# seshnadathur/victor

Measured on AMD Instinct MI355X. Metric: likelihood evals/sec (40 s-bins, 100 mu, l=0,2,4), higher is better.
Workload: dtype f64

## Files before the change

### victor_amd/csrc/vk_devmath.h

```cpp
#pragma once

#include <hip/hip_runtime.h>

namespace vkm {

template <int CTRL, int ROW_MASK, bool BOUND_CTRL = false>
__device__ __forceinline__ double dpp_move(double v) {
  int lo = __double2loint(v), hi = __double2hiint(v);
  lo = __builtin_amdgcn_update_dpp(0, lo, CTRL, ROW_MASK, 0xF, BOUND_CTRL);
  hi = __builtin_amdgcn_update_dpp(0, hi, CTRL, ROW_MASK, 0xF, BOUND_CTRL);
  return __hiloint2double(hi, lo);
}

__device__ __forceinline__ double wave_sum(double v) {
  v += dpp_move<0xB1, 0xF, true>(v);
  v += dpp_move<0x4E, 0xF, true>(v);
  v += dpp_move<0x141, 0xF, true>(v);
  v += dpp_move<0x140, 0xF, true>(v);
  v += dpp_move<0x142, 0xF, true>(v);
  v += dpp_move<0x143, 0xF, true>(v);
  const int lo = __builtin_amdgcn_readlane(__double2loint(v), 63);
  const int hi = __builtin_amdgcn_readlane(__double2hiint(v), 63);
  return __hiloint2double(hi, lo);
}

__device__ __forceinline__ double fold32(double x, double y) {
  const auto lo = __builtin_amdgcn_permlane32_swap((unsigned)__double2loint(x), (unsigned)__double2loint(y), false, false);
  const auto hi = __builtin_amdgcn_permlane32_swap((unsigned)__double2hiint(x), (unsigned)__double2hiint(y), false, false);
  return __hiloint2double((int)hi[0], (int)lo[0]) + __hiloint2double((int)hi[1], (int)lo[1]);
}
__device__ __forceinline__ double fold16(double x, double y) {
  const auto lo = __builtin_amdgcn_permlane16_swap((unsigned)__double2loint(x), (unsigned)__double2loint(y), false, false);
  const auto hi = __builtin_amdgcn_permlane16_swap((unsigned)__double2hiint(x), (unsigned)__double2hiint(y), false, false);
  return __hiloint2double((int)hi[0], (int)lo[0]) + __hiloint2double((int)hi[1], (int)lo[1]);
}
__device__ __forceinline__ double octet_sum(double v) {
  v += dpp_move<0x141, 0xF, true>(v);
  v += dpp_move<0xB1, 0xF, true>(v);
  v += dpp_move<0x4E, 0xF, true>(v);
  return v;
}

__device__ __forceinline__ void sqrt_rsqrt(double x, double& g, double& ir) {
  const double y = __builtin_amdgcn_rsq(x);
  const double e = fma(-(x * y), y, 1.0);
  const double p = fma(0.375, e, 0.5);
  ir = fma(y * e, p, y);
  g = x * ir;
}

__device__ __forceinline__ double rsqrt3(double x) {
  const double y = __builtin_amdgcn_rsq(x);
  const double e = fma(-(x * y), y, 1.0);
  const double p = fma(0.375, e, 0.5);
  return fma(y * e, p, y);
}

__device__ __forceinline__ double rsqrt_nr(double x) {
  const double y = __builtin_amdgcn_rsq(x);
  const double e = fma(-(x * y), y, 1.0);
  return fma(y * e, 0.5, y);
}

__device__ __forceinline__ double recip(double x) {
  const double y = __builtin_amdgcn_rcp(x);
  const double e = fma(-x, y, 1.0);
  return fma(y, fma(e, e, e), y);
}

constexpr int kExpNonposTab = 256;
__device__ __forceinline__ double exp2_frac(int j) { return exp2((double)j * (1.0 / kExpNonposTab)); }

__device__ __forceinline__ double fma3(double p, double f, double c) {
  double r;
  asm("v_fma_f64 %0, %1, %2, %3" : "=v"(r) : "v"(p), "v"(f), "v"(c));
  return r;
}

__device__ __forceinline__ double exp_nonpos(double a, const double* __restrict__ tab) {
  a = fmax(a, -750.0);
  const double n = rint(a * 369.3299304675746);
  double f = fma(n, -0x1.62e42fee00000p-9, a);
  f = fma(n, -0x1.a39ef35793c76p-41, f);
  const int ni = (int)n;
  const double t = tab[ni & (kExpNonposTab - 1)];
  double p = fma3(f, 1.0 / 24.0, 1.0 / 6.0);
  p = fma(p, f, 0.5);
  p = fma(p, f, 1.0);
  p = fma(p, f, 1.0);
  return ldexp(t * p, ni >> 8);
}

__device__ __forceinline__ double fma_s(double p, double f, double c) {
  double r;
  asm("v_fma_f64 %0, %1, %2, %3" : "=v"(r) : "v"(p), "v"(f), "s"(c));
  return r;
}

__device__ __forceinline__ double recip_nr(double x) {
  const double y = __builtin_amdgcn_rcp(x);
  const double e = fma(-x, y, 1.0);
  return fma(y, e, y);
}

__device__ __forceinline__ void recip_shared2(double a, double b, double& ra, double& rb) {
  const double P = a * b;
  const double y = recip(P);
  ra = y * b;
  rb = y * a;
}
__device__ __forceinline__ void recip_shared3(double a, double b, double c, double& ra, double& rb, double& rc) {
  const double ab = a * b;
  const double P = ab * c;
  const double y = recip(P);
  const double yc = y * c;
  rc = y * ab;
  ra = yc * b;
  rb = yc * a;
}
__device__ __forceinline__ void recip_shared4(double a, double b, double c, double d, double& ra, double& rb, double& rc, double& rd) {
  const double ab = a * b, cd = c * d;
  const double P = ab * cd;
  const double y = recip(P);
  const double yab = y * ab;
  const double ycd = y * cd;
  ra = ycd * b;
  rb = ycd * a;
  rc = yab * d;
  rd = yab * c;
}

__device__ __forceinline__ double rsqrt_nr_x2(double x) {
  const double y = __builtin_amdgcn_rsq(x);
  const double h = x * y;
  const double w = fma(-h, y, 3.0);
  return y * w;
}

__device__ __forceinline__ double rsqrt3_x2(double x) {
  const double y = __builtin_amdgcn_rsq(x);
  const double e = fma(-(x * y), y, 1.0);
  const double p2 = fma(0.75, e, 1.0);
  return y * fma(e, p2, 2.0);
}

constexpr double kExpScale = 13.589148804608305 * 0x1p-9;
constexpr double kExpC = 709.782712893383996843;
template <int EXPT> struct ExpCfg;
template <> struct ExpCfg<0> {
  static constexpr int kBits = 8, kEntries = 256, kDoubles = 256, kDegree = 3;
  static constexpr double kMagic = 0x1.8p34;
  static constexpr double kLead = kExpC * kExpC * kExpC / 6.0;
};
template <> struct ExpCfg<1> {
  static constexpr int kBits = 6, kEntries = 64, kDoubles = 64 * 32, kDegree = 4;
  static constexpr double kMagic = 0x1.8p36;
  static constexpr double kLead = kExpC * kExpC * kExpC * kExpC / 24.0;
};
constexpr int kExpTab = ExpCfg<0>::kDoubles;

template <int EXPT>
__device__ __forceinline__ double exp_table_entry(int j) {
  typedef ExpCfg<EXPT> C;
  const double t = C::kLead * exp2((double)j * (1.0 / C::kEntries));
  return __hiloint2double(__double2hiint(t) - (j << (20 - C::kBits)), __double2loint(t));
}
template <int EXPT>
__device__ __forceinline__ double exp_table_slot(int e) { return exp_table_entry<EXPT>(EXPT == 1 ? (e >> 5) : e); }

__device__ __forceinline__ void clamp_keeps_nan() { asm volatile("s_setreg_imm32_b32 hwreg(HW_REG_MODE, 8, 1), 0"); }

template <int EXPT>
__device__ __forceinline__ double exp_gauss(double ynum, double inv_sv, const double* __restrict__ tab, unsigned lane_off = 0) {
  typedef ExpCfg<EXPT> C;
  double yp;
  asm("v_mul_f64 %0, |%1|, |%2| clamp" : "=v"(yp) : "v"(ynum), "v"(inv_sv));
  const double nd = fma(-yp, yp, C::kMagic);
  const double nn = nd - C::kMagic;
  const double d = fma(-yp, yp, -nn);
  const int n = __double2loint(nd);
  unsigned off;
  if (EXPT == 0) {
    asm("v_lshlrev_b32_sdwa %0, %1, %2 dst_sel:DWORD dst_unused:UNUSED_PAD src0_sel:DWORD src1_sel:BYTE_0" : "=v"(off) : "v"(3), "v"(n));
    __builtin_assume(off < 2048u);
  } else {
    asm("v_and_b32 %0, 63, %1\n\tv_lshl_or_b32 %0, %0, 8, %2" : "=&v"(off) : "v"(n), "v"(lane_off));
  }
  (void)tab;
  double t;
  asm("ds_read_b64 %0, %1\n\ts_waitcnt lgkmcnt(0)" : "=v"(t) : "v"(off));
  const double ts = __hiloint2double(__double2hiint(t) + (n << (20 - C::kBits)), __double2loint(t));
  double q;
  if (C::kDegree == 3) {
    q = d + 3.0 / kExpC;
    q = fma_s(q, d, 6.0 / (kExpC * kExpC));
    q = fma_s(q, d, 6.0 / (kExpC * kExpC * kExpC));
  } else {
    q = d + 4.0 / kExpC;
    q = fma_s(q, d, 12.0 / (kExpC * kExpC));
    q = fma_s(q, d, 24.0 / (kExpC * kExpC * kExpC));
    q = fma_s(q, d, 24.0 / (kExpC * kExpC * kExpC * kExpC));
  }
  return ts * q;
}

}
```

### victor_amd/csrc/vk_kernel_cells.h

```cpp
#pragma once
#include "vk_kernel_fast.h"

namespace vk {

struct CellsPlan {
  int mu, w, s, betar, da, v1, sva, image_end, acc, like, total;
};

__host__ __device__ inline int cells_range_bins(int n_mu, int cpi) { return (cpi + n_mu - 2) / n_mu + 1; }

__host__ __device__ inline CellsPlan make_cells_plan(int n_mu, int n_x, int n_s, int uni_n, int nlr, int n_beta_r,
                                                     int lut_n, int with_da, int cpi, int n_like, int n_sva = 0) {
  CellsPlan p;
  int o = fast_fixed_doubles(uni_n, nlr, lut_n);
  o = (o + 1) & ~1;
  p.mu = o;    o += 2 * n_mu;
  p.w = o;     o += kMaxEll * n_mu;
  p.s = o;     o += (n_s + 1) & ~1;
  p.betar = o; o += (n_beta_r + 1) & ~1;
  p.da = o;    o += with_da ? uni_n * 4 : 0;
  p.v1 = o;    o += with_da == 1 ? 0 : uni_n * 4;
  o = (o + 1) & ~1;
  p.sva = o;   o += (n_sva + 1) & ~1;
  p.image_end = o;
  int bins = cells_range_bins(n_mu, cpi);
  if (bins > n_s) bins = n_s;
  p.acc = o;   o += kMaxEll * (bins + 1) * kWaves;
  o = (o + 1) & ~1;
  p.like = o;  o += n_like > 0 ? like_lds_doubles(n_like) : 0;
  p.total = o;
  return p;
}

template <int NLR>
__device__ __forceinline__ void stage_cells(const TheoryArgs& a, const CellsPlan& pl, double* lds, int with_da) {
  const int tid = threadIdx.x;
  for (int i = tid; i < a.n_mu; i += kBlock) {
    const double m = a.mu[i];
    lds[pl.mu + 2 * i] = m;
    lds[pl.mu + 2 * i + 1] = sqrt(1.0 - m * m);
#pragma unroll
    for (int l = 0; l < kMaxEll; ++l) lds[pl.w + l * a.n_mu + i] = (l < a.n_ell) ? a.w_ell[l * a.n_mu + i] : 0.0;
  }
  for (int j = tid; j < a.n_s; j += kBlock) lds[pl.s + j] = a.s[j];
  stage_uni_records<NLR>(a, lds);
  if (with_da) stage_da<NLR>(a, lds + pl.da);
  if (with_da != 1) for (int e = tid; e < a.uni_n * 4; e += kBlock) lds[pl.v1 + e] = a.uni_sv_v[(e >> 2) * 8 + 4 + (e & 3)];
  if (a.n_beta_r > 0)
    for (int i = tid; i < a.n_beta_r; i += kBlock) lds[pl.betar + i] = a.beta_r[i];
  if (pl.image_end > pl.sva)
    for (int e = tid; e < a.sva_doubles; e += kBlock) lds[pl.sva + e] = a.sva[e];
}

template <int NL>
__device__ __forceinline__ void finish_point_ranges(const TheoryArgs& a, long long point, double beta, double poison, double* th,
                                                    bool gather, const double* lds_beta_r) {
  const int N = a.n_ell * a.n_s;
  const double w0 = a.wsum[0], w1 = a.wsum[1], w2 = a.wsum[2];
  const bool keep_out = !a.fuse || a.want_theory;
  LikePrefetch<kLikeRowsCells> pf;
  if (a.fuse) pf.issue(a.like, beta, late_tid(), lds_beta_r);
  for (int e = late_tid(); gather && e < N; e += kBlock) {
    const int l = (e >= 2 * a.n_s) ? 2 : (e >= a.n_s ? 1 : 0), j = e - l * a.n_s;
    const int q_first = (j * a.n_mu) / a.cells_per_item, q_last = (j * a.n_mu + a.n_mu - 1) / a.cells_per_item;
    double part[8];
    load_shared_x8(partial_slot(a, point, l, j), part);
    double v = 0.0;
#pragma unroll
    for (int c = 0; c < kMaxParts; ++c) v += (c <= q_last - q_first) ? part[c] : 0.0;
    v = v - (l == 0 ? w0 : (l == 1 ? w1 : w2)) + poison;
    if (keep_out) a.out[point * (long long)N + e] = v;
    th[e] = v;
  }
  __syncthreads();
  if (a.fuse) like_point_workgroup(a.like, point, beta, th, th + like_red_off(N), pf);
}

__device__ __forceinline__ double uniform_f64(double v) {
  return __hiloint2double(__builtin_amdgcn_readfirstlane(__double2hiint(v)), __builtin_amdgcn_readfirstlane(__double2loint(v)));
}

template <int NL>
__device__ __forceinline__ void project_trip(double g, bool first, bool second, const double* w_i, int n_mu, double* acc, int lstride, int lane) {
  const double ga = first ? g : 0.0, gb = second ? g : 0.0;
  double z[NL];
#pragma unroll
  for (int l = 0; l < NL; ++l) {
    const double w = w_i[l * n_mu];
    z[l] = vkm::fold32(w * ga, w * gb);
  }
  double x;
  int l_mine;
  bool mine;
  const int row = lane >> 4;
  if (NL == 3) {
    const double u = vkm::fold16(z[0], z[1]);
    const double v = vkm::fold16(z[2], 0.0);
    const bool up = (lane & 8) != 0;
    const double keep = up ? v : u, send = up ? u : v;
    x = keep + vkm::dpp_move<0x128, 0xF, true>(send);
    l_mine = up ? 2 : (row & 1);
    mine = (lane & 7) == 0 && !(up && (row & 1));
  } else {
    x = vkm::fold16(z[0], NL == 2 ? z[NL - 1] : 0.0);
    x += vkm::dpp_move<0x128, 0xF, true>(x);
    l_mine = row & 1;
    mine = (lane & 15) == 0 && (NL == 2 || !(row & 1));
  }
  x = vkm::octet_sum(x);
  if (mine) acc[l_mine * lstride + (lane >> 5) * kWaves] += x;
}

constexpr int kNodeBlock = 4;

template <int W, int NLR, int GRID, int FD, int CL, int SVA>
__device__ __forceinline__ void stream_block(const double* __restrict__ lds, const FastConsts& fc, const FastPoint& fp, double s_par,
                                             double sperp2, double sperp2x, const VelocityNode (&c)[kNodeBlock], double& g, double& gs) {
  UniHead h[W];
  double inv[W], p[W];
#pragma unroll
  for (int i = 0; i < W; ++i) {
    h[i] = uni_point_head<NLR, GRID, FD, 1, CL, 0, SVA>(lds, fc, 0.0, fma(-c[i].x, fp.Bk, s_par), sperp2, c[i].x, fp.fa, sperp2x);
    asm volatile("" : "+v"(h[i].SV), "+v"(h[i].ynum), "+v"(h[i].xi1));
    __builtin_amdgcn_sched_barrier(0);
  }
  if (W == 4) vkm::recip_shared4(h[0].SV, h[1 % W].SV, h[2 % W].SV, h[3 % W].SV, inv[0], inv[1 % W], inv[2 % W], inv[3 % W]);
  if (W == 3) vkm::recip_shared3(h[0].SV, h[1 % W].SV, h[2 % W].SV, inv[0], inv[1 % W], inv[2 % W]);
  if (W == 2) vkm::recip_shared2(h[0].SV, h[1 % W].SV, inv[0], inv[1 % W]);
  if (W == 1) inv[0] = vkm::recip_nr(h[0].SV);
#pragma unroll
  for (int i = 0; i < W; ++i) p[i] = uni_point_tail<0>(lds, h[i], inv[i], 0u);
#pragma unroll
  for (int i = 0; i < W; ++i) {
    gs = fma(inv[i], p[i], gs);
    if (c[i].last != 0) {
      asm volatile("" ::: "memory");
      g = fma(c[i].w, gs, g);
      gs = 0.0;
    }
  }
}

template <int NLR, int GRID, int FD, int CL, int SVA>
__device__ __forceinline__ double stream_cell(const TheoryArgs& a, const double* __restrict__ lds, const FastConsts& fc, const FastPoint& fp,
                                              double s_par, double sperp2, double sperp2x) {
  constexpr int W = kNodeBlock;
  double g = 0.0, gs = 0.0;
  const double* xgw = a.xgw;
  asm volatile("" : "+s"(xgw));
  VelocityNode nx[W];
#pragma unroll
  for (int i = 0; i < W; ++i) nx[i] = load_node(xgw, i);
  const int quads = a.n_xg / W;
  for (int b = 0; b < quads; ++b) {
    VelocityNode c[W];
#pragma unroll
    for (int i = 0; i < W; ++i) c[i] = nx[i];
#pragma unroll
    for (int i = 0; i < W; ++i) nx[i] = load_node(xgw, W * b + W + i);
    stream_block<W, NLR, GRID, FD, CL, SVA>(lds, fc, fp, s_par, sperp2, sperp2x, c, g, gs);
  }
  const int rest = a.n_xg - quads * W;
  if (rest == 3) stream_block<3, NLR, GRID, FD, CL, SVA>(lds, fc, fp, s_par, sperp2, sperp2x, nx, g, gs);
  else if (rest == 2) stream_block<2, NLR, GRID, FD, CL, SVA>(lds, fc, fp, s_par, sperp2, sperp2x, nx, g, gs);
  else if (rest == 1) stream_block<1, NLR, GRID, FD, CL, SVA>(lds, fc, fp, s_par, sperp2, sperp2x, nx, g, gs);
  return g;
}

template <int NLR, int NL, int GRID, int MODE, int SVA = 0>
__global__ __launch_bounds__(kBlock, (MODE == kModeStreaming && !SVA) || MODE == kModeKaiser ? 5 : 4) void vk_theory_cells_kernel(TheoryArgs a) {
  extern __shared__ double lds[];
  vkm::clamp_keeps_nan();
  warm_kernarg_lines<sizeof(TheoryArgs)>();
  const int N = a.n_ell * a.n_s;
  const int R = a.parts;
  const int cpi = a.cells_per_item;
  const bool xi_out = NL == 1 && a.xi_out != 0;
  const bool tail = !xi_out && (a.fuse || R > 1);
  CellsPlan pl = make_cells_plan(a.n_mu, a.n_x, a.n_s, a.uni_n, NLR, a.n_beta_r, a.uni_lut_n, mode_layout(MODE), xi_out ? 0 : cpi,
                                 tail ? N : 0, SVA ? a.sva_doubles : 0);
  pl.like = __builtin_amdgcn_readfirstlane(pl.like);
  const int tid = threadIdx.x;
  VK_STAMP(a, 0);
  if (a.image) copy_image(lds, a.image, pl.image_end);
  else stage_cells<NLR>(a, pl, lds, mode_layout(MODE));
  constexpr bool kHalf = MODE != kModeKaiser;
  const FastConsts fc = make_fast_consts<NLR>(a, kHalf, SVA ? pl.sva : 0);
  __syncthreads();
  VK_STAMP(a, 1);

  const int lane = tid & 63;
  const int wave = __builtin_amdgcn_readfirstlane(tid >> 6);
  const double* l_mu = lds + pl.mu;
  const double* l_w = lds + pl.w;
  const double* l_s = lds + pl.s;
  const int slots = xi_out ? 1 : min(cells_range_bins(a.n_mu, cpi), a.n_s) + 1;
  double* l_acc = lds + pl.acc;
  const unsigned items = (unsigned)a.n * (unsigned)R;
  const int all_cells = a.n_s * a.n_mu;

  {
    const unsigned item = blockIdx.x;
    if (item >= items) return;
    const long long point = item / (unsigned)R;
    const int q = (int)(item - (unsigned)point * (unsigned)R);
    const int c0 = q * cpi, c1 = min(c0 + cpi, all_cells);
    const int jf = (int)__umulhi((unsigned)c0, a.nmu_magic);
    const int nb = (int)__umulhi((unsigned)(c1 - 1), a.nmu_magic) - jf + 1;
    const double* row = a.params + point * VK_NPAR;
    constexpr bool kStream = !mode_has_da(MODE);
    PointScalars ps = point_scalars(a, row);
    if (kStream) ps.poison = uniform_f64(ps.poison);
    FastPoint fp = make_fast_point(ps, fc, kHalf);
    if (kStream) {
      fp.k_perp = uniform_f64(fp.k_perp);
      fp.k_par = uniform_f64(fp.k_par);
    }
    const double xi_max = kStream ? uniform_f64(a.xw_max * fabs(fp.Bk)) : 0.0;
    const double rlo2 = kStream ? uniform_f64(fc.rlo2) : 0.0, rhi2 = kStream ? uniform_f64(fc.rhi2) : 0.0;
    FastConsts fcs = fc;
    if (kStream && GRID == 0) {
      fcs.off = uniform_f64(fc.off);
      fcs.t_lo = uniform_f64(fc.t_lo);
      fcs.n_eps = uniform_f64(fc.n_eps);
    }
    constexpr int PV = MODE == kModeKaiser ? 0 : 1;
    __syncthreads();
    rebuild_point_tables<NLR, PV>(a, lds, pl.betar, pl.v1, row[VK_P_BETA], ps.av, mode_is_dispersion(MODE) ? -fp.Gk : fp.AVk,
                                  mode_has_da(MODE) ? lds + pl.da : nullptr);
    if (mode_has_da(MODE) && a.empirical && !a.vr_beta_dep) rebuild_da_emp(a, lds + pl.da, ps.av);
    for (int e = lane; e < kMaxEll * slots; e += 64) l_acc[e * kWaves + wave] = 0.0;
    __syncthreads();
    VK_STAMP(a, 2);
    for (int base = c0 + 64 * wave; base < c1; base += 64 * kWaves) {
      auto cell_of = [&](int e_, bool& live_, int& i_, int& j_) {
        live_ = e_ < c1;
        const unsigned ec = (unsigned)(live_ ? e_ : c1 - 1);
        const int hi = xi_out ? (a.n_s == 1 ? (int)ec : (int)__umulhi(ec, a.ns_magic)) : (int)__umulhi(ec, a.nmu_magic);
        const int lo = (int)ec - hi * (xi_out ? a.n_s : a.n_mu);
        j_ = xi_out ? lo : hi;
        i_ = xi_out ? hi : lo;
      };
      int i0, j;
      bool live0;
      cell_of(base + lane, live0, i0, j);
      const double sj = l_s[j];
      const vk_d2 mm = *reinterpret_cast<const vk_d2*>(l_mu + 2 * i0);
      const double s_perp = sj * fp.k_perp * mm.y;
      const double sperp2 = s_perp * s_perp;
      const double sperp2x = sperp2 * fp.fp2;
      const double s_par = sj * fp.k_par * mm.x;
      double g = 0.0;
      const bool inside = kStream && !__any(!cell_in_table(rlo2, rhi2, s_par, sperp2, xi_max));
      double gs = 0.0;
      if (MODE == kModeKaiser) {
        g = kaiser_value<NLR, GRID>(lds, lds + pl.da, fc, fp, ps.M, ps.Q, a.niter, a.coord_shift != 0, a.kaiser_approx != 0,
                                    a.rsd == VK_RSD_EUCLID, a.from_data != 0, s_par, sperp2);
      } else if (mode_is_dispersion(MODE)) {
        const double inv_den0 = disp_first_pass<NLR, GRID>(lds, fc, fp, a.niter, s_par, sperp2);
        for (int k = 0; k < a.n_xg; ++k) {
          const VelocityNode xw = load_node(a.xgw, k);
          gs += disp_value<NLR, GRID, MODE == kModeDispersionFromData, SVA>(lds, lds + pl.da, fc, fp, a.niter, fma(-xw.x, fp.Bk, s_par), inv_den0,
                                                                     sperp2, xw.x);
          if (xw.last != 0) {
            asm volatile("" ::: "memory");
            g = fma(xw.w, gs, g);
            gs = 0.0;
          }
        }
      } else if (inside) {
        g = stream_cell<NLR, GRID, MODE == kModeFromData, 0, SVA>(a, lds, fcs, fp, s_par, sperp2, sperp2x);
      } else {
        g = stream_cell<NLR, GRID, MODE == kModeFromData, GRID == 0 ? 2 : 1, SVA>(a, lds, fcs, fp, s_par, sperp2, sperp2x);
      }
      const int lane2 = kStream ? late_tid() & 63 : lane;
      const int e = base + lane2;
      int i = i0, j2 = j;
      bool live = live0;
      if (kStream) cell_of(e, live, i, j2);
      if (xi_out) {
        if (live) a.out[point * (long long)all_cells + e] = g - 1.0 + ps.poison;
        continue;
      }
      const int jj = j2 - jf;
      const int jj0 = __builtin_amdgcn_readfirstlane(jj);
      project_trip<NL>(g, live && jj == jj0, live && jj != jj0, l_w + i, a.n_mu, l_acc + jj0 * kWaves + wave, slots * kWaves, lane2);
    }
    if (xi_out) return;
    __syncthreads();
    double* th = lds + pl.like;
    for (int e = late_tid(); e < NL * nb; e += kBlock) {
      const int l = e / nb, jl = e - l * nb;
      const int j = jf + jl;
      const double* pa = l_acc + (l * slots + jl) * kWaves;
      const double sum = (pa[0] + pa[1]) + (pa[2] + pa[3]);
      if (R > 1) {
        store_shared(partial_slot(a, point, l, j) + (q - (j * a.n_mu) / cpi), sum);
      } else {
        const double v = sum - (l == 0 ? a.wsum[0] : (l == 1 ? a.wsum[1] : a.wsum[2])) + ps.poison;
        if (!a.fuse || a.want_theory) a.out[point * (long long)N + l * a.n_s + j] = v;
        if (tail) th[l * a.n_s + j] = v;
      }
    }
    VK_STAMP(a, 3);
    if (tail) {
      bool last = true;
      if (R > 1) {
        int* flag = reinterpret_cast<int*>(th + like_red_off(N) + kLikeRed + 2);
        last = point_completed(a.counters, point, (unsigned)R, flag);
      }
      VK_STAMP(a, 4);
      if (last) {
        finish_point_ranges<NL>(a, point, row[VK_P_BETA], ps.poison, th, R > 1, a.n_beta_r > 0 ? lds + pl.betar : nullptr);
        VK_STAMP(a, 5);
      }
      return;
    }
  }
}


}
```

### victor_amd/csrc/vk_kernel_fast.h

```cpp
#pragma once
#include "vk_common.h"
#include "vk_kernel_like.h"

namespace vk {

typedef double vk_d2 __attribute__((ext_vector_type(2)));
constexpr int kMuRec = 6;
constexpr int kEtabOff = 0;
template <int EXPT> __host__ __device__ constexpr int recs_off() { return vkm::ExpCfg<EXPT>::kDoubles; }
__host__ __device__ constexpr int recs_off_rt(int expt) { return expt ? vkm::ExpCfg<1>::kDoubles : vkm::ExpCfg<0>::kDoubles; }

__host__ __device__ constexpr int uni_stride(int nlr) { return 4 * (2 + nlr) + 2; }
__host__ __device__ constexpr int fast_fixed_doubles(int uni_n, int nlr, int lut_n, int expt = 0) {
  return recs_off_rt(expt) + (uni_n + (lut_n > 0 ? 2 : 0)) * uni_stride(nlr) + (lut_n + 3) / 4;
}

struct FastConsts {
  double inv_h;
  double off, t_lo, n_eps;
  double inv_g;
  double rlo2, rhi2;
  int lut_off;
  double sv_a, sv_b, sv_tmax;
  double mu_lo, mu_hi, mu_inv_h;
// ... 121 lines not shown

template <int NLR>
__device__ __forceinline__ void rebuild_uni_xi(const TheoryArgs& a, double* recs, const double* bg, double beta, double vs = 1.0,
                                               double av = 0.0, double* da = nullptr) {
  constexpr int stride = uni_stride(NLR);
  const int tid = late_tid();
  int kb = 0;
  if (a.n_beta_r <= 64) {
    const int lane = tid & 63;
    kb = __popcll(__ballot(lane >= 1 && lane < a.n_beta_r - 1 && beta >= bg[lane < a.n_beta_r ? lane : 0]));
  } else {
    for (int i = 1; i < a.n_beta_r - 1; ++i) kb = (beta >= bg[i]) ? i : kb;
  }
  const double db = beta - bg[kb];
  const int per_l = a.uni_n * 4;
  const size_t stride_l = (size_t)(a.n_beta_r - 1) * per_l * 4;
  const double* src = ((NLR > 1) ? a.uni_xic : a.uni_xi) + (size_t)kb * per_l * 4;
  const int total = NLR * per_l;
  for (int base = tid; base < total; base += 4 * kBlock) {
    vk_d2 c01[4], c23[4];
#pragma unroll
    for (int k = 0; k < 4; ++k) {
      const int e = min(base + k * kBlock, total - 1);
      const int l = (NLR > 2 && e >= 2 * per_l) ? 2 : ((NLR > 1 && e >= per_l) ? 1 : 0);
      const double* c = src + l * stride_l + (size_t)(e - l * per_l) * 4;
      c01[k] = *reinterpret_cast<const vk_d2*>(c);
      c23[k] = *reinterpret_cast<const vk_d2*>(c + 2);
    }
#pragma unroll
    for (int k = 0; k < 4; ++k) {
      const int e = base + k * kBlock;
      if (e < total) {
        const int l = (NLR > 2 && e >= 2 * per_l) ? 2 : ((NLR > 1 && e >= per_l) ? 1 : 0);
        const int iq = e - l * per_l;
        recs[(iq >> 2) * stride + 8 + 4 * l + (iq & 3)] = fma(fma(fma(c23[k].y, db, c23[k].x), db, c01[k].y), db, c01[k].x);
      }
    }
  }
  if (a.vr_beta_dep) {
    const size_t var6 = (size_t)(a.n_beta_r - 1) * per_l * 7;
    const double* e6 = a.uni_empb + (size_t)kb * per_l * 7;
    for (int iq = tid; iq < per_l; iq += kBlock) {
      const double* c = a.uni_vb + ((size_t)kb * per_l + iq) * 4;
      double v = fma(fma(fma(c[3], db, c[2]), db, c[1]), db, c[0]);
      if (a.empirical) v = fma(av, poly6(e6 + (size_t)iq * 7, db), v);
      recs[(iq >> 2) * stride + 4 + (iq & 3)] = vs * v;
      if (da) {
        if (a.empirical) {
          da[iq] = fma(av, poly6(e6 + 2 * var6 + (size_t)iq * 7, db), poly6(e6 + var6 + (size_t)iq * 7, db));
        } else {
          const double* d = a.uni_dab + ((size_t)kb * per_l + iq) * 4;
          da[iq] = fma(fma(fma(d[3], db, d[2]), db, d[1]), db, d[0]);
        }
      }
    }
  }
}

template <int NLR>
__device__ __forceinline__ void rebuild_uni_v_emp(const TheoryArgs& a, double* recs, double av, double vs = 1.0) {
  constexpr int stride = uni_stride(NLR);
  for (int iq = late_tid(); iq < a.uni_n * 4; iq += kBlock)
    recs[(iq >> 2) * stride + 4 + (iq & 3)] = vs * fma(av, a.uni_v2[iq], a.uni_sv_v[(iq >> 2) * 8 + 4 + (iq & 3)]);
}

template <int NLR>
__device__ __forceinline__ void scale_uni_v(int uni_n, double* recs, const double* v1, double vs) {
  constexpr int stride = uni_stride(NLR);
  for (int iq = late_tid(); iq < uni_n * 4; iq += kBlock) recs[(iq >> 2) * stride + 4 + (iq & 3)] = vs * v1[iq];
}

template <int NLR, int PV>
__device__ __forceinline__ void rebuild_point_tables(const TheoryArgs& a, double* lds, int betar_off, int v1_off, double beta,
                                                     double av, double AVk, double* da = nullptr) {
  const double vs = PV ? AVk : 1.0;
  double* recs = lds + recs_off<0>();
  if (a.n_beta_r > 0) rebuild_uni_xi<NLR>(a, recs, lds + betar_off, beta, vs, av, a.vr_beta_dep ? da : nullptr);
  if (a.empirical && !a.vr_beta_dep) rebuild_uni_v_emp<NLR>(a, recs, av, vs);
  else if (PV && !a.vr_beta_dep) scale_uni_v<NLR>(a.uni_n, recs, lds + v1_off, vs);
}

struct FastPoint {
  double fa, fp2;
  double Gk, gD;
  double k_perp, k_par;
  double Bk;
  double AVk;
};

__device__ __forceinline__ FastPoint make_fast_point(const PointScalars& ps, const FastConsts& fc, bool half) {
  FastPoint fp;
  const double hs = half ? 0.5 : 1.0;
  const double k = ps.inv_c * fc.inv_h;
  const double kl = k * hs;
  fp.k_perp = ps.aperp * kl;
  fp.k_par = ps.apar * kl;
  fp.Bk = ps.B * kl * (1.0 / vkm::kExpScale);
  fp.AVk = ps.A * vkm::kExpScale * hs;
  const double c = 1.0 / ps.inv_c;
  fp.fa = c * ps.inv_apar;
  fp.fp2 = (c * ps.inv_aperp) * (c * ps.inv_aperp);
  fp.Gk = ps.G * k * (half ? 0.25 : 1.0);
  fp.gD = ps.gD;
  return fp;
}

template <int NLR, int GRID, int CL = 1, int EXPT = 0>
__device__ __forceinline__ const double* locate(const double* __restrict__ lds, const FastConsts& fc, double x,
                                                double& tq, int& qi) {
  constexpr int stride = uni_stride(NLR);
  constexpr int roff = recs_off<EXPT>();
  if (GRID == 0) {
    const double t = CL == 2 ? vmin_f64_s(vmax_f64_s(x, fc.t_lo), fc.n_eps) : (CL ? vmin_f64(vmax_f64(x, fc.t_lo), fc.n_eps) : x);
    tq = __builtin_amdgcn_fract(t);
    qi = (int)t;
    return lds_at(lds + roff, __mul24(qi, stride * 8));
  }
  const double u = CL ? vmin_f64(vmax_f64(x, fc.t_lo), fc.n_eps) : x;
  const int cell = (int)(u * fc.inv_g);
  const int q0 = *reinterpret_cast<const unsigned short*>(reinterpret_cast<const char*>(lds) + fc.lut_off + 2 * cell);
  const double* rec0 = lds_at(lds + roff, __mul24(q0, stride * 8));
  const double k1 = rec0[2 * stride - 2], k2 = rec0[3 * stride - 2];
  const int q = q0 + (u >= k1) + (u >= k2);
  qi = q;
  const double* rec = lds_at(lds + roff, __mul24(q, stride * 8));
  const vk_d2 kw = *reinterpret_cast<const vk_d2*>(rec + stride - 2);
  tq = (u - kw.x) * kw.y;
  return rec;
}

__device__ __forceinline__ double sv_aniso(const double* __restrict__ lds, const FastConsts& fc, double rp, double mu2) {
  const double ts = vmin_f64(vmax_f64(fma(rp, fc.sv_a, fc.sv_b), 0.0), fc.sv_tmax);
  const double du = __builtin_amdgcn_fract(ts);
  const int i = (int)ts;
  const double m = vmin_f64(vmax_f64(0.5 * mu2, fc.mu_lo), fc.mu_hi);
  const double* muk = lds_at(lds, fc.svmu_off);
  int j;
  if (fc.mu_inv_h > 0.0) {
    j = min((int)((m - fc.mu_lo) * fc.mu_inv_h), fc.sv_nm - 1);
  } else {
    j = 0;
    for (int k = 1; k < fc.sv_nm; ++k) j += (m >= muk[k]) ? 1 : 0;
  }
  const double dm = m - muk[j];
  const double* c = lds_at(lds, fc.sva_off + (i * fc.sv_nm + j) * 128);
  double acc = cubic_b128(c + 12, dm);
  acc = fma(acc, du, cubic_b128(c + 8, dm));
  acc = fma(acc, du, cubic_b128(c + 4, dm));
  return fma(acc, du, cubic_b128(c, dm));
}

struct UniHead { double SV, ynum, xi1; };

template <int NLR, int GRID, int FD, int PV = 0, int CL = 1, int EXPT = 0, int SVA = 0>
__device__ __forceinline__ UniHead uni_point_head(const double* __restrict__ lds, const FastConsts& fc, double AVh,
                                                  double num, double sperp2, double xk, double fa, double sperp2x) {
  const double X = fma(num, num, sperp2);
  const double yy = vkm::rsqrt_nr_x2(X);
  const double mu2 = num * yy;
  double mu_x = mu2;
  double tq;
  int qi;
  const double rp = SVA ? X * yy : 0.0;
  const double* rec = locate<NLR, GRID, CL, EXPT>(lds, fc, GRID == 0 ? (SVA ? rp + fc.off : fma(X, yy, fc.off)) : X * yy, tq, qi);
  const double SV = SVA ? sv_aniso(lds, fc, rp, mu2) : cubic_b128(rec, tq);
  const double V = cubic_b128(rec + 4, tq);
  const double ynum = PV ? fma(V, mu2, xk) : fma(AVh * V, mu2, xk);
  if (FD) {
    const double rp = num * fa;
    const double Xx = fma(rp, rp, sperp2x);
    const double yyx = vkm::rsqrt_nr_x2(Xx);
    mu_x = rp * yyx;
    rec = locate<NLR, GRID, CL == 2 ? 2 : 1, EXPT>(lds, fc, GRID == 0 ? fma(Xx, yyx, fc.off) : Xx * yyx, tq, qi);
  }
  double xi1 = cubic_b128(rec + 8, tq);
  if (NLR > 1) {
    const double m2 = mu_x * mu_x;
    if (NLR == 2) {
      xi1 = fma(cubic_b128(rec + 12, tq), m2, xi1);
    } else {
      xi1 = fma(fma(cubic_b128(rec + 16, tq), m2, cubic_b128(rec + 12, tq)), m2, xi1);
    }
  }
  UniHead h;
  h.SV = SV;
  h.ynum = ynum;
  h.xi1 = xi1;
  return h;
}

template <int EXPT = 0>
__device__ __forceinline__ double uni_point_tail(const double* __restrict__ lds, const UniHead& h, double inv_sv, unsigned lane_off) {
  const double e = vkm::exp_gauss<EXPT>(h.ynum, inv_sv, lds + kEtabOff, lane_off);
  return e * h.xi1;
}

template <int NLR, int GRID, int FD, int PV = 0, int CL = 1, int EXPT = 0, int SVA = 0>
__device__ __forceinline__ double uni_point(const double* __restrict__ lds, const FastConsts& fc, double AVh,
                                            double num, double sperp2, double xk, double fa, double sperp2x,
                                            unsigned lane_off, double& inv_sv) {
  const UniHead h = uni_point_head<NLR, GRID, FD, PV, CL, EXPT, SVA>(lds, fc, AVh, num, sperp2, xk, fa, sperp2x);
  inv_sv = vkm::recip_nr(h.SV);
  return uni_point_tail<EXPT>(lds, h, inv_sv, lane_off);
}

template <int NLR, int GRID>
__device__ __forceinline__ double disp_first_pass(const double* __restrict__ lds, const FastConsts& fc, const FastPoint& fp,
                                                  int niter, double s_par, double sperp2) {
  double tq;
  int qi;
  const bool last = niter == 0;
  const double X = fma(s_par, s_par, sperp2);
  const double yy = last ? vkm::rsqrt3_x2(X) : vkm::rsqrt_nr_x2(X);
  const double* rec = locate<NLR, GRID>(lds, fc, GRID == 0 ? fma(X, yy, fc.off) : X * yy, tq, qi);
  const double den = fma(cubic_b128(rec + 4, tq), yy, 1.0);
  return last ? vkm::recip(den) : vkm::recip_nr(den);
}

template <int NLR, int GRID, int FD, int SVA = 0>
__device__ __forceinline__ double disp_value(const double* __restrict__ lds, const double* __restrict__ da,
                                             const FastConsts& fc, const FastPoint& fp, int niter, double num,
                                             double inv_den0, double sperp2, double xk) {
  double tq;
  int qi;
  auto pass = [&](double rp, bool last) {
    const double X = fma(rp, rp, sperp2);
    const double yy = last ? vkm::rsqrt3_x2(X) : vkm::rsqrt_nr_x2(X);
    const double* rec = locate<NLR, GRID>(lds, fc, GRID == 0 ? fma(X, yy, fc.off) : X * yy, tq, qi);
    const double den = fma(cubic_b128(rec + 4, tq), yy, 1.0);
    return num * (last ? vkm::recip(den) : vkm::recip_nr(den));
  };
  double r_par = num * inv_den0;
  for (int it = __builtin_amdgcn_readfirstlane(niter) - 1; it > 0; --it) r_par = pass(r_par, false);
  if (niter >= 1) r_par = pass(r_par, true);
  const double X = fma(r_par, r_par, sperp2);
  const double yy = vkm::rsqrt3_x2(X);
  const double mu2 = r_par * yy;
  const double rp = SVA ? X * yy : 0.0;
  const double* rec = locate<NLR, GRID>(lds, fc, GRID == 0 ? (SVA ? rp + fc.off : fma(X, yy, fc.off)) : X * yy, tq, qi);
  const double SV = SVA ? sv_aniso(lds, fc, rp, mu2) : cubic_b128(rec, tq);
  const double q = cubic_b128(rec + 4, tq) * yy;
  const double dq = -fp.gD * cubic_b128(da + 4 * qi, tq);
  double mx2 = mu2 * mu2;
  const double m2 = 0.25 * mx2;
  if (FD) {
    const double rpx = r_par * fp.fa;
    const double Xx = fma(rpx, rpx, sperp2 * fp.fp2);
    const double yyx = vkm::rsqrt3_x2(Xx);
    const double mu_x = rpx * yyx;
    mx2 = mu_x * mu_x;
    rec = locate<NLR, GRID>(lds, fc, GRID == 0 ? fma(Xx, yyx, fc.off) : Xx * yyx, tq, qi);
  }
  double xi1 = cubic_b128(rec + 8, tq);
  if (NLR == 2) xi1 = fma(cubic_b128(rec + 12, tq), mx2, xi1);
  if (NLR == 3) xi1 = fma(fma(cubic_b128(rec + 16, tq), mx2, cubic_b128(rec + 12, tq)), mx2, xi1);
  const double inv_sv = vkm::recip(SV);
  const double jac = vkm::recip(1.0 + q + m2 * (dq - q));
  const double e = vkm::exp_gauss<0>(xk, inv_sv, lds + kEtabOff);
  return inv_sv * jac * (e * xi1);
}

template <int NLR, int GRID>
__device__ __forceinline__ double kaiser_value(const double* __restrict__ lds, const double* __restrict__ da, const FastConsts& fc,
                                               const FastPoint& fp, double M, double Q, int niter, bool coord_shift, bool linear,
                                               bool euclid, bool fd, double s_par, double sperp2) {
  double tq;
  int qi;
  const double MG = -M * fp.Gk;
  auto pass = [&](double rp, bool last) {
    const double r2 = fma(rp, rp, sperp2);
    const double inv_r = last ? vkm::rsqrt3(r2) : vkm::rsqrt_nr(r2);
    const double* rec = locate<NLR, GRID>(lds, fc, GRID == 0 ? fma(r2, inv_r, fc.off) : r2 * inv_r, tq, qi);
    const double den = fma(cubic_b128(rec + 4, tq) * inv_r, MG, 1.0);
    return s_par * (last ? vkm::recip(den) : vkm::recip_nr(den));
  };
  double r_par = s_par;
  if (coord_shift) {
    for (int it = 0; it < niter; ++it) r_par = pass(r_par, false);
    r_par = pass(r_par, true);
  }
  const double r2 = fma(r_par, r_par, sperp2);
  const double inv_r = vkm::rsqrt3(r2);
  const double mu_r = r_par * inv_r;
  const double* rec = locate<NLR, GRID>(lds, fc, GRID == 0 ? fma(r2, inv_r, fc.off) : r2 * inv_r, tq, qi);
  const double q = -fp.Gk * cubic_b128(rec + 4, tq) * inv_r;
  const double dq = -fp.gD * cubic_b128(da + 4 * qi, tq);
  const double m2 = mu_r * mu_r;
  double mx2 = 4.0 * m2;
  if (fd) {
    const double rp = r_par * fp.fa;
    const double r2x = fma(rp, rp, sperp2 * fp.fp2);
    const double inv_rx = vkm::rsqrt3(r2x);
    const double mu_x = rp * inv_rx;
    mx2 = 4.0 * (mu_x * mu_x);
    rec = locate<NLR, GRID>(lds, fc, GRID == 0 ? fma(r2x, inv_rx, fc.off) : r2x * inv_rx, tq, qi);
  }
  double xi1 = cubic_b128(rec + 8, tq);
  if (NLR == 2) xi1 = fma(cubic_b128(rec + 12, tq), mx2, xi1);
  if (NLR == 3) xi1 = fma(fma(cubic_b128(rec + 16, tq), mx2, cubic_b128(rec + 12, tq)), mx2, xi1);
  const double mxi = M * (xi1 - 1.0);
  const double J = euclid ? 3.0 * M * q + 2.0 * M * Q * m2 * (dq - q) : M * q + M * Q * m2 * (dq - q);
  if (linear || euclid) return 1.0 + (mxi - J);
  return (1.0 + mxi) * vkm::recip(1.0 + J);
}

constexpr int kModeStreaming = 0, kModeFromData = 1, kModeDispersion = 2, kModeDispersionFromData = 3, kModeKaiser = 4;
__host__ __device__ constexpr bool mode_is_dispersion(int mode) { return mode == kModeDispersion || mode == kModeDispersionFromData; }
__host__ __device__ constexpr bool mode_has_da(int mode) { return mode >= kModeDispersion; }
__host__ __device__ constexpr int mode_layout(int mode) { return mode_is_dispersion(mode) ? 2 : (mode_has_da(mode) ? 1 : 0); }

template <int NLR>
__device__ __forceinline__ void stage_da(const TheoryArgs& a, double* da) {
  if (!a.uni_da) return;
  for (int e = threadIdx.x; e < a.uni_n * 4; e += kBlock) da[e] = a.uni_da[e];
}

__device__ __forceinline__ void rebuild_da_emp(const TheoryArgs& a, double* da, double av) {
  const int n4 = a.uni_n * 4;
  for (int e = threadIdx.x; e < n4; e += kBlock) da[e] = fma(av, a.uni_ge[n4 + e], a.uni_ge[e]);
}


__device__ __forceinline__ double* partial_slot(double* partial, int n_s, long long point, int l, int j) {
  return partial + (((point * kMaxEll + l) * n_s + j) * (long long)kMaxParts);
}
__device__ __forceinline__ double* partial_slot(const TheoryArgs& a, long long point, int l, int j) {
  return partial_slot(a.partial, a.n_s, point, l, j);
}

template <int NL, int RB = kLikeRows>
__device__ __forceinline__ void finish_point(const TheoryArgs& a, long long point, double beta, double poison, double* th,
                                             bool gather_partials, const double* lds_beta_r, bool poll = false) {
  const int N = a.n_ell * a.n_s;
  double* red = th + like_red_off(N);
  const double w0 = a.wsum[0], w1 = a.wsum[1], w2 = a.wsum[2];
  LikePrefetch<RB> pf;
  if (a.fuse) pf.issue(a.like, beta, late_tid(), lds_beta_r);
  for (int e = threadIdx.x; e < N; e += kBlock) {
    double v;
    if (gather_partials) {
      const int l = (e >= 2 * a.n_s) ? 2 : (e >= a.n_s ? 1 : 0), j = e - l * a.n_s;
// ... 266 lines not shown
```

Before: 2.770 million.

## Software-pipeline LDS table reads and exp lookups in stream_block

Splits the per-point head into a geometry stage and an LDS-read stage, so that in the common GRID==0, non-FD, non-SVA path the next point's geometry and reads overlap the current point's cubic evaluations. The exp table lookup is split into issue, polynomial and wait stages with graded lgkmcnt waits, letting all W ds_reads be in flight together. The next node global loads are moved after the head phase through a callback. The aim is to hide LDS latency, at the cost of more live registers and fragile hand-written waitcnt ordering.

```diff
diff --git a/victor_amd/csrc/vk_devmath.h b/victor_amd/csrc/vk_devmath.h
--- a/victor_amd/csrc/vk_devmath.h
+++ b/victor_amd/csrc/vk_devmath.h
@@ -171,25 +171,24 @@
 __device__ __forceinline__ void clamp_keeps_nan() { asm volatile("s_setreg_imm32_b32 hwreg(HW_REG_MODE, 8, 1), 0"); }
 
 template <int EXPT>
-__device__ __forceinline__ double exp_gauss(double ynum, double inv_sv, const double* __restrict__ tab, unsigned lane_off = 0) {
+__device__ __forceinline__ void exp_gauss_reduce(double ynum, double inv_sv, unsigned lane_off, double& d, int& n, unsigned& off) {
   typedef ExpCfg<EXPT> C;
   double yp;
   asm("v_mul_f64 %0, |%1|, |%2| clamp" : "=v"(yp) : "v"(ynum), "v"(inv_sv));
   const double nd = fma(-yp, yp, C::kMagic);
   const double nn = nd - C::kMagic;
-  const double d = fma(-yp, yp, -nn);
-  const int n = __double2loint(nd);
-  unsigned off;
+  d = fma(-yp, yp, -nn);
+  n = __double2loint(nd);
   if (EXPT == 0) {
     asm("v_lshlrev_b32_sdwa %0, %1, %2 dst_sel:DWORD dst_unused:UNUSED_PAD src0_sel:DWORD src1_sel:BYTE_0" : "=v"(off) : "v"(3), "v"(n));
     __builtin_assume(off < 2048u);
   } else {
     asm("v_and_b32 %0, 63, %1\n\tv_lshl_or_b32 %0, %0, 8, %2" : "=&v"(off) : "v"(n), "v"(lane_off));
   }
-  (void)tab;
-  double t;
-  asm("ds_read_b64 %0, %1\n\ts_waitcnt lgkmcnt(0)" : "=v"(t) : "v"(off));
-  const double ts = __hiloint2double(__double2hiint(t) + (n << (20 - C::kBits)), __double2loint(t));
+}
+template <int EXPT>
+__device__ __forceinline__ double exp_gauss_poly(double d) {
+  typedef ExpCfg<EXPT> C;
   double q;
   if (C::kDegree == 3) {
     q = d + 3.0 / kExpC;
@@ -201,7 +200,51 @@
     q = fma_s(q, d, 24.0 / (kExpC * kExpC * kExpC));
     q = fma_s(q, d, 24.0 / (kExpC * kExpC * kExpC * kExpC));
   }
-  return ts * q;
-}
-
-}
+  return q;
+}
+template <int EXPT>
+__device__ __forceinline__ double exp_gauss_scale(double t, int n) {
+  return __hiloint2double(__double2hiint(t) + (n << (20 - ExpCfg<EXPT>::kBits)), __double2loint(t));
+}
+
+template <int EXPT> struct ExpPending {
+  double d, t;
+  int n;
+};
+template <int EXPT>
+__device__ __forceinline__ ExpPending<EXPT> exp_gauss_issue(double ynum, double inv_sv, const double* __restrict__ tab, unsigned lane_off = 0) {
+  ExpPending<EXPT> e;
+  unsigned off;
+  exp_gauss_reduce<EXPT>(ynum, inv_sv, lane_off, e.d, e.n, off);
+  (void)tab;
+  asm volatile("ds_read_b64 %0, %1" : "=v"(e.t) : "v"(off));
+  return e;
+}
+template <int EXPT>
+__device__ __forceinline__ void exp_gauss_wait(ExpPending<EXPT>& e, int newer) {
+  switch (newer) {
+    case 3: asm volatile("s_waitcnt lgkmcnt(3)" : "+v"(e.t)); break;
+    case 2: asm volatile("s_waitcnt lgkmcnt(2)" : "+v"(e.t)); break;
+    case 1: asm volatile("s_waitcnt lgkmcnt(1)" : "+v"(e.t)); break;
+    default: asm volatile("s_waitcnt lgkmcnt(0)" : "+v"(e.t)); break;
+  }
+}
+template <int EXPT>
+__device__ __forceinline__ double exp_gauss_finish(const ExpPending<EXPT>& e, double q) {
+  return exp_gauss_scale<EXPT>(e.t, e.n) * q;
+}
+
+template <int EXPT>
+__device__ __forceinline__ double exp_gauss(double ynum, double inv_sv, const double* __restrict__ tab, unsigned lane_off = 0) {
+  double d;
+  int n;
+  unsigned off;
+  exp_gauss_reduce<EXPT>(ynum, inv_sv, lane_off, d, n, off);
+  (void)tab;
+  double t;
+  asm("ds_read_b64 %0, %1\n\ts_waitcnt lgkmcnt(0)" : "=v"(t) : "v"(off));
+  const double ts = exp_gauss_scale<EXPT>(t, n);
+  return ts * exp_gauss_poly<EXPT>(d);
+}
+
+}
diff --git a/victor_amd/csrc/vk_kernel_cells.h b/victor_amd/csrc/vk_kernel_cells.h
--- a/victor_amd/csrc/vk_kernel_cells.h
+++ b/victor_amd/csrc/vk_kernel_cells.h
@@ -113,23 +113,58 @@
 
 constexpr int kNodeBlock = 4;
 
-template <int W, int NLR, int GRID, int FD, int CL, int SVA>
+template <int W, int NLR, int GRID, int FD, int CL, int SVA, typename NEXT>
 __device__ __forceinline__ void stream_block(const double* __restrict__ lds, const FastConsts& fc, const FastPoint& fp, double s_par,
-                                             double sperp2, double sperp2x, const VelocityNode (&c)[kNodeBlock], double& g, double& gs) {
+                                             double sperp2, double sperp2x, const VelocityNode (&c)[kNodeBlock], double& g, double& gs,
+                                             NEXT&& fetch_next) {
   UniHead h[W];
   double inv[W], p[W];
-#pragma unroll
-  for (int i = 0; i < W; ++i) {
-    h[i] = uni_point_head<NLR, GRID, FD, 1, CL, 0, SVA>(lds, fc, 0.0, fma(-c[i].x, fp.Bk, s_par), sperp2, c[i].x, fp.fa, sperp2x);
-    asm volatile("" : "+v"(h[i].SV), "+v"(h[i].ynum), "+v"(h[i].xi1));
+  constexpr bool kTwoDeep = GRID == 0 && !FD && !SVA;
+  if (kTwoDeep) {
+    UniGeo geo = uni_head_geometry<NLR, GRID, CL>(lds, fc, fma(-c[0].x, fp.Bk, s_par), sperp2);
+    UniRecs<NLR> recs = uni_head_reads<NLR>(geo);
     __builtin_amdgcn_sched_barrier(0);
-  }
+#pragma unroll
+    for (int i = 0; i < W; ++i) {
+      UniGeo next = geo;
+      if (i + 1 < W) {
+        next = uni_head_geometry<NLR, GRID, CL>(lds, fc, fma(-c[(i + 1) % W].x, fp.Bk, s_par), sperp2);
+        asm volatile("" : "+v"(next.tq), "+v"(next.mu2));
+        __builtin_amdgcn_sched_barrier(0);
+      }
+      h[i] = uni_head_cubics_of<NLR>(recs, geo, c[i].x);
+      asm volatile("" : "+v"(h[i].SV), "+v"(h[i].ynum), "+v"(h[i].xi1));
+      __builtin_amdgcn_sched_barrier(0);
+      if (i + 1 < W) {
+        geo = next;
+        recs = uni_head_reads<NLR>(geo);
+        __builtin_amdgcn_sched_barrier(0);
+      }
+    }
+  } else {
+#pragma unroll
+    for (int i = 0; i < W; ++i) {
+      h[i] = uni_point_head<NLR, GRID, FD, 1, CL, 0, SVA>(lds, fc, 0.0, fma(-c[i].x, fp.Bk, s_par), sperp2, c[i].x, fp.fa, sperp2x);
+      asm volatile("" : "+v"(h[i].SV), "+v"(h[i].ynum), "+v"(h[i].xi1));
+      __builtin_amdgcn_sched_barrier(0);
+    }
+  }
+  fetch_next();
   if (W == 4) vkm::recip_shared4(h[0].SV, h[1 % W].SV, h[2 % W].SV, h[3 % W].SV, inv[0], inv[1 % W], inv[2 % W], inv[3 % W]);
   if (W == 3) vkm::recip_shared3(h[0].SV, h[1 % W].SV, h[2 % W].SV, inv[0], inv[1 % W], inv[2 % W]);
   if (W == 2) vkm::recip_shared2(h[0].SV, h[1 % W].SV, inv[0], inv[1 % W]);
   if (W == 1) inv[0] = vkm::recip_nr(h[0].SV);
-#pragma unroll
-  for (int i = 0; i < W; ++i) p[i] = uni_point_tail<0>(lds, h[i], inv[i], 0u);
+  vkm::ExpPending<0> e[W];
+  double q[W];
+#pragma unroll
+  for (int i = 0; i < W; ++i) e[i] = vkm::exp_gauss_issue<0>(h[i].ynum, inv[i], lds + kEtabOff);
+#pragma unroll
+  for (int i = 0; i < W; ++i) q[i] = vkm::exp_gauss_poly<0>(e[i].d);
+#pragma unroll
+  for (int i = 0; i < W; ++i) {
+    vkm::exp_gauss_wait(e[i], W - 1 - i);
+    p[i] = vkm::exp_gauss_finish(e[i], q[i]) * h[i].xi1;
+  }
 #pragma unroll
   for (int i = 0; i < W; ++i) {
     gs = fma(inv[i], p[i], gs);
@@ -156,14 +191,15 @@
     VelocityNode c[W];
 #pragma unroll
     for (int i = 0; i < W; ++i) c[i] = nx[i];
-#pragma unroll
-    for (int i = 0; i < W; ++i) nx[i] = load_node(xgw, W * b + W + i);
-    stream_block<W, NLR, GRID, FD, CL, SVA>(lds, fc, fp, s_par, sperp2, sperp2x, c, g, gs);
+    stream_block<W, NLR, GRID, FD, CL, SVA>(lds, fc, fp, s_par, sperp2, sperp2x, c, g, gs, [&]() {
+#pragma unroll
+      for (int i = 0; i < W; ++i) nx[i] = load_node(xgw, W * b + W + i);
+    });
   }
   const int rest = a.n_xg - quads * W;
-  if (rest == 3) stream_block<3, NLR, GRID, FD, CL, SVA>(lds, fc, fp, s_par, sperp2, sperp2x, nx, g, gs);
-  else if (rest == 2) stream_block<2, NLR, GRID, FD, CL, SVA>(lds, fc, fp, s_par, sperp2, sperp2x, nx, g, gs);
-  else if (rest == 1) stream_block<1, NLR, GRID, FD, CL, SVA>(lds, fc, fp, s_par, sperp2, sperp2x, nx, g, gs);
+  if (rest == 3) stream_block<3, NLR, GRID, FD, CL, SVA>(lds, fc, fp, s_par, sperp2, sperp2x, nx, g, gs, []() {});
+  else if (rest == 2) stream_block<2, NLR, GRID, FD, CL, SVA>(lds, fc, fp, s_par, sperp2, sperp2x, nx, g, gs, []() {});
+  else if (rest == 1) stream_block<1, NLR, GRID, FD, CL, SVA>(lds, fc, fp, s_par, sperp2, sperp2x, nx, g, gs, []() {});
   return g;
 }
 
diff --git a/victor_amd/csrc/vk_kernel_fast.h b/victor_amd/csrc/vk_kernel_fast.h
--- a/victor_amd/csrc/vk_kernel_fast.h
+++ b/victor_amd/csrc/vk_kernel_fast.h
@@ -297,18 +297,33 @@
 
 struct UniHead { double SV, ynum, xi1; };
 
-template <int NLR, int GRID, int FD, int PV = 0, int CL = 1, int EXPT = 0, int SVA = 0>
-__device__ __forceinline__ UniHead uni_point_head(const double* __restrict__ lds, const FastConsts& fc, double AVh,
-                                                  double num, double sperp2, double xk, double fa, double sperp2x) {
+struct UniGeo {
+  const double* rec;
+  double tq, mu2;
+  double rp;
+};
+
+template <int NLR, int GRID, int CL = 1, int EXPT = 0, int SVA = 0>
+__device__ __forceinline__ UniGeo uni_head_geometry(const double* __restrict__ lds, const FastConsts& fc, double num, double sperp2) {
+  UniGeo g;
   const double X = fma(num, num, sperp2);
   const double yy = vkm::rsqrt_nr_x2(X);
-  const double mu2 = num * yy;
+  g.mu2 = num * yy;
+  int qi;
+  g.rp = SVA ? X * yy : 0.0;
+  g.rec = locate<NLR, GRID, CL, EXPT>(lds, fc, GRID == 0 ? (SVA ? g.rp + fc.off : fma(X, yy, fc.off)) : X * yy, g.tq, qi);
+  return g;
+}
+
+template <int NLR, int GRID, int FD, int PV = 0, int CL = 1, int EXPT = 0, int SVA = 0>
+__device__ __forceinline__ UniHead uni_head_cubics(const double* __restrict__ lds, const FastConsts& fc, const UniGeo& g, double AVh,
+                                                   double num, double xk, double fa, double sperp2x) {
+  const double mu2 = g.mu2;
   double mu_x = mu2;
-  double tq;
+  double tq = g.tq;
   int qi;
-  const double rp = SVA ? X * yy : 0.0;
-  const double* rec = locate<NLR, GRID, CL, EXPT>(lds, fc, GRID == 0 ? (SVA ? rp + fc.off : fma(X, yy, fc.off)) : X * yy, tq, qi);
-  const double SV = SVA ? sv_aniso(lds, fc, rp, mu2) : cubic_b128(rec, tq);
+  const double* rec = g.rec;
+  const double SV = SVA ? sv_aniso(lds, fc, g.rp, mu2) : cubic_b128(rec, tq);
   const double V = cubic_b128(rec + 4, tq);
   const double ynum = PV ? fma(V, mu2, xk) : fma(AVh * V, mu2, xk);
   if (FD) {
@@ -332,6 +347,70 @@
   h.ynum = ynum;
   h.xi1 = xi1;
   return h;
+}
+
+template <int NLR> struct UniRecs { vk_d2 sv_hi, sv_lo, v_hi, v_lo, xi[NLR][2]; };
+
+template <int NLR>
+__device__ __forceinline__ void uni_head_reads_sv_v(const UniGeo& g, UniRecs<NLR>& r) {
+  const vk_d2* rec = reinterpret_cast<const vk_d2*>(g.rec);
+  r.sv_hi = rec[1];
+  r.v_hi = rec[3];
+  r.sv_lo = rec[0];
+  r.v_lo = rec[2];
+}
+template <int NLR>
+__device__ __forceinline__ void uni_head_reads_xi(const UniGeo& g, UniRecs<NLR>& r) {
+  const vk_d2* rec = reinterpret_cast<const vk_d2*>(g.rec);
+#pragma unroll
+  for (int l = NLR - 1; l >= 0; --l) {
+    r.xi[l][0] = rec[4 + 2 * l + 1];
+    r.xi[l][1] = rec[4 + 2 * l];
+  }
+}
+template <int NLR>
+__device__ __forceinline__ UniRecs<NLR> uni_head_reads(const UniGeo& g) {
+  UniRecs<NLR> r;
+  uni_head_reads_sv_v<NLR>(g, r);
+  uni_head_reads_xi<NLR>(g, r);
+  return r;
+}
+
+__device__ __forceinline__ double cubic_pairs(const vk_d2& hi, const vk_d2& lo, double t) {
+  return fma(fma(fma(hi.y, t, hi.x), t, lo.y), t, lo.x);
+}
+
+template <int NLR>
+__device__ __forceinline__ void uni_head_cubics_sv_v(const UniRecs<NLR>& r, const UniGeo& g, double xk, UniHead& h) {
+  h.SV = cubic_pairs(r.sv_hi, r.sv_lo, g.tq);
+  h.ynum = fma(cubic_pairs(r.v_hi, r.v_lo, g.tq), g.mu2, xk);
+}
+template <int NLR>
+__device__ __forceinline__ void uni_head_cubics_xi(const UniRecs<NLR>& r, const UniGeo& g, UniHead& h) {
+  double xi1 = cubic_pairs(r.xi[0][0], r.xi[0][1], g.tq);
+  if (NLR > 1) {
+    const double m2 = g.mu2 * g.mu2;
+    if (NLR == 2) {
+      xi1 = fma(cubic_pairs(r.xi[1][0], r.xi[1][1], g.tq), m2, xi1);
+    } else {
+      xi1 = fma(fma(cubic_pairs(r.xi[2][0], r.xi[2][1], g.tq), m2, cubic_pairs(r.xi[1][0], r.xi[1][1], g.tq)), m2, xi1);
+    }
+  }
+  h.xi1 = xi1;
+}
+template <int NLR>
+__device__ __forceinline__ UniHead uni_head_cubics_of(const UniRecs<NLR>& r, const UniGeo& g, double xk) {
+  UniHead h;
+  uni_head_cubics_sv_v<NLR>(r, g, xk, h);
+  uni_head_cubics_xi<NLR>(r, g, h);
+  return h;
+}
+
+template <int NLR, int GRID, int FD, int PV = 0, int CL = 1, int EXPT = 0, int SVA = 0>
+__device__ __forceinline__ UniHead uni_point_head(const double* __restrict__ lds, const FastConsts& fc, double AVh,
+                                                  double num, double sperp2, double xk, double fa, double sperp2x) {
+  const UniGeo g = uni_head_geometry<NLR, GRID, CL, EXPT, SVA>(lds, fc, num, sperp2);
+  return uni_head_cubics<NLR, GRID, FD, PV, CL, EXPT, SVA>(lds, fc, g, AVh, num, xk, fa, sperp2x);
 }
 
 template <int EXPT = 0>
```

After: 2.784 million (median of 6 runs). No clear change (+0.5%).

## Give each wave a contiguous cell run and reduce projections once per s-bin

Applied to the files above, without the earlier changes.

Changes how cells are split across waves: each wave now takes one contiguous run of cells instead of interleaving 64-cell strides with the other waves. Multipole projections are kept in per-lane register accumulators and cross-lane folded only when the s-bin changes, replacing a DPP/octet reduction on every 64-cell trip. The aim is to cut the cross-lane reduction and LDS accumulation work. The new path is disabled by a constexpr predicate for some streaming and Kaiser configurations. It costs extra registers and can leave waves unevenly loaded when run lengths differ.

```diff
diff --git a/victor_amd/csrc/vk_kernel_cells.h b/victor_amd/csrc/vk_kernel_cells.h
--- a/victor_amd/csrc/vk_kernel_cells.h
+++ b/victor_amd/csrc/vk_kernel_cells.h
@@ -81,14 +81,10 @@
 }
 
 template <int NL>
-__device__ __forceinline__ void project_trip(double g, bool first, bool second, const double* w_i, int n_mu, double* acc, int lstride, int lane) {
-  const double ga = first ? g : 0.0, gb = second ? g : 0.0;
+__device__ __forceinline__ void fold_bins(const double (&za)[NL], const double (&zb)[NL], double* acc, int lstride, int lane) {
   double z[NL];
 #pragma unroll
-  for (int l = 0; l < NL; ++l) {
-    const double w = w_i[l * n_mu];
-    z[l] = vkm::fold32(w * ga, w * gb);
-  }
+  for (int l = 0; l < NL; ++l) z[l] = vkm::fold32(za[l], zb[l]);
   double x;
   int l_mine;
   bool mine;
@@ -111,6 +107,43 @@
   if (mine) acc[l_mine * lstride + (lane >> 5) * kWaves] += x;
 }
 
+template <int NL>
+__device__ __forceinline__ void project_trip(double g, bool first, bool second, const double* w_i, int n_mu, double* acc, int lstride, int lane) {
+  const double ga = first ? g : 0.0, gb = second ? g : 0.0;
+  double za[NL], zb[NL];
+#pragma unroll
+  for (int l = 0; l < NL; ++l) {
+    const double w = w_i[l * n_mu];
+    za[l] = w * ga;
+    zb[l] = w * gb;
+  }
+  fold_bins<NL>(za, zb, acc, lstride, lane);
+}
+
+template <int NL>
+__device__ __forceinline__ void accumulate_trip(double g, bool first, bool second, const double* w_i, int n_mu, double (&za)[NL], double (&zb)[NL]) {
+  const double ga = first ? g : 0.0, gb = second ? g : 0.0;
+#pragma unroll
+  for (int l = 0; l < NL; ++l) {
+    const double w = w_i[l * n_mu];
+    za[l] = fma(w, ga, za[l]);
+    zb[l] = fma(w, gb, zb[l]);
+  }
+}
+
+template <int NL>
+__device__ __forceinline__ void fold_bin(const double (&za)[NL], double* acc, int lstride, int lane) {
+  const int row = lane >> 4;
+  const double u = vkm::fold32(za[0], za[NL >= 2 ? 1 : 0]);
+  const double v = NL == 3 ? vkm::fold32(za[NL - 1], za[NL - 1]) : u;
+  double x = vkm::fold16(u, v);
+  x += vkm::dpp_move<0x128, 0xF, true>(x);
+  x = vkm::octet_sum(x);
+  const int l_mine = NL == 3 ? (row == 1 ? 2 : row >> 1) : row >> 1;
+  const bool mine = (lane & 15) == 0 && (NL == 3 ? row != 3 : !(row & 1) && (NL == 2 || row == 0));
+  if (mine) acc[l_mine * lstride] += x;
+}
+
 constexpr int kNodeBlock = 4;
 
 template <int W, int NLR, int GRID, int FD, int CL, int SVA>
@@ -165,6 +198,13 @@
   else if (rest == 2) stream_block<2, NLR, GRID, FD, CL, SVA>(lds, fc, fp, s_par, sperp2, sperp2x, nx, g, gs);
   else if (rest == 1) stream_block<1, NLR, GRID, FD, CL, SVA>(lds, fc, fp, s_par, sperp2, sperp2x, nx, g, gs);
   return g;
+}
+
+template <int NLR, int NL, int GRID, int MODE, int SVA>
+constexpr bool cells_project_per_bin() {
+  if (GRID == 1 && MODE == kModeStreaming && !SVA && NLR == 3 && NL >= 2) return false;
+  if (GRID == 1 && MODE == kModeKaiser && NLR >= 2 && NL == 3) return false;
+  return true;
 }
 
 template <int NLR, int NL, int GRID, int MODE, int SVA = 0>
@@ -232,7 +272,15 @@
     for (int e = lane; e < kMaxEll * slots; e += 64) l_acc[e * kWaves + wave] = 0.0;
     __syncthreads();
     VK_STAMP(a, 2);
-    for (int base = c0 + 64 * wave; base < c1; base += 64 * kWaves) {
+    constexpr bool kPerBin = cells_project_per_bin<NLR, NL, GRID, MODE, SVA>();
+    const int run_cells = 64 * ((((c1 - c0 + 63) >> 6) + kWaves - 1) / kWaves);
+    const int t0 = kPerBin ? c0 + run_cells * wave : c0 + 64 * wave;
+    const int t1 = kPerBin ? min(t0 + run_cells, c1) : c1;
+    double za[NL], zb[NL];
+#pragma unroll
+    for (int l = 0; l < NL; ++l) za[l] = zb[l] = 0.0;
+    int cur = kPerBin && !xi_out ? (int)__umulhi((unsigned)min(t0, c1 - 1), a.nmu_magic) - jf : 0;
+    for (int base = t0; base < t1; base += kPerBin ? 64 : 64 * kWaves) {
       auto cell_of = [&](int e_, bool& live_, int& i_, int& j_) {
         live_ = e_ < c1;
         const unsigned ec = (unsigned)(live_ ? e_ : c1 - 1);
@@ -284,9 +332,24 @@
       }
       const int jj = j2 - jf;
       const int jj0 = __builtin_amdgcn_readfirstlane(jj);
-      project_trip<NL>(g, live && jj == jj0, live && jj != jj0, l_w + i, a.n_mu, l_acc + jj0 * kWaves + wave, slots * kWaves, lane2);
+      if (kPerBin) {
+        if (jj0 != cur) {
+          asm volatile("" ::: "memory");
+          fold_bin<NL>(za, l_acc + cur * kWaves + wave, slots * kWaves, lane2);
+#pragma unroll
+          for (int l = 0; l < NL; ++l) {
+            za[l] = zb[l];
+            zb[l] = 0.0;
+          }
+          cur = jj0;
+        }
+        accumulate_trip<NL>(g, live && jj == jj0, live && jj != jj0, l_w + i, a.n_mu, za, zb);
+      } else {
+        project_trip<NL>(g, live && jj == jj0, live && jj != jj0, l_w + i, a.n_mu, l_acc + jj0 * kWaves + wave, slots * kWaves, lane2);
+      }
     }
     if (xi_out) return;
+    if (kPerBin && t0 < t1) fold_bins<NL>(za, zb, l_acc + cur * kWaves + wave, slots * kWaves, kStream ? late_tid() & 63 : lane);
     __syncthreads();
     double* th = lds + pl.like;
     for (int e = late_tid(); e < NL * nb; e += kBlock) {
```

Result: no change. 2.849 million before, 2.860 million after, median of 6 (+0.4%).
